# toonsegers/verifiable_mpc

Measured on AMD Instinct MI355X. Metric: Ed25519 MSM scalar-mults/sec, higher is better.
Workload: dtype u32 (255-bit modular integers as 10 limbs of 25.5 bits, 32x32->64 multiply-adds)

## Files before the change

verifiable_mpc_amd/csrc/msm.hip:

```cpp
#include <stdlib.h>

#include "common.h"
#include "fe25519.h"
#include "fr.h"
#include "ge25519.h"
#include "scan.h"
#include "quad.h"
#include "msm_sort.h"
#include "ptio.h"

#ifndef MSM_NIELS_STRIDE
#define MSM_NIELS_STRIDE 24
#endif
#ifndef MSM_REDUCE_WAVES
#define MSM_REDUCE_WAVES 2
#endif

__global__ void __launch_bounds__(MSM_BLOCK)
k_msm_prep(const uint32_t *__restrict__ aff, size_t n_main, const uint32_t *__restrict__ aff_extra,
           size_t n_total, uint32_t *__restrict__ niels) {
    size_t i = (size_t)blockIdx.x * blockDim.x + threadIdx.x;
    if (i >= n_total) return;
    const uint32_t *src = (i < n_main) ? aff + 16 * i : aff_extra + 16 * (i - n_main);
    ge_aff a;
// ... 364 lines not shown

extern "C" int vmpc_msm_dev(vmpc_ctx *ctx, const void *scalars, const void *affine_points, size_t n,
                            const void *extra_scalars, const void *extra_affine_points,
                            size_t n_extra, void *out_ext, void *out_affine) {
    if (!ctx || (n && (!scalars || !affine_points)) || (n_extra && (!extra_scalars || !extra_affine_points)))
        return VMPC_E_INVAL;
    if (!out_ext && !out_affine) return VMPC_E_INVAL;
    VMPC_HIP_CHECK(hipSetDevice(ctx->device));
    hipStream_t st = ctx->stream;
    size_t n_total = n + n_extra;
    if (n_total == 0) {
        uint32_t id_ext[32] = {0}, id_aff[16] = {0};
        id_ext[8] = 1; id_ext[16] = 1; id_aff[8] = 1;
        if (out_ext) VMPC_HIP_CHECK(hipMemcpyAsync(out_ext, id_ext, 128, hipMemcpyHostToDevice, st));
        if (out_affine) VMPC_HIP_CHECK(hipMemcpyAsync(out_affine, id_aff, 64, hipMemcpyHostToDevice, st));
        VMPC_HIP_CHECK(hipStreamSynchronize(st));
        return VMPC_OK;
    }
    if (n_total >= (1ull << 31) / 16) return VMPC_E_INVAL;
    msm_plan p;
    msm_make_plan(ctx, n, n_extra, 253, p, &ED25519_L);
    msm_ws w;
    msm_layout(p, w, nullptr, NIELS_WORDS * 4, EXT_WORDS * 4);
    VMPC_CHECK(vmpc_ws_reserve(ctx, w.total));
    msm_layout(p, w, (char *)ctx->ws, NIELS_WORDS * 4, EXT_WORDS * 4);

    {
        vmpc_stage_scope s(ctx, "msm_prep");
        k_msm_prep<<<(unsigned)((n_total + MSM_BLOCK - 1) / MSM_BLOCK), MSM_BLOCK, 0, st>>>(
            (const uint32_t *)affine_points, n, (const uint32_t *)extra_affine_points, n_total, w.entries);
        VMPC_KERNEL_CHECK();
    }
    VMPC_CHECK(msm_sort_stage(ctx, p, w, scalars, n, extra_scalars, ED25519_L));
    return msm_accumulate(ctx, p, w, w.entries, out_ext, out_affine);
}

bool msm_short_fits(const vmpc_ctx *ctx, size_t table_n, size_t table_extra, size_t m, int rows, int c, int K,
                    const void *out_ext, const void *out_affine);
int msm_short_batch(vmpc_ctx *ctx, const void *table, size_t table_n, size_t table_extra, const void *const *scalars,
                    size_t m, const void *const *extra_scalars, int K, void *out_ext, const msm_modulus &modulus);

static int msm_table_window(const vmpc_ctx *ctx) {
    const int o = ctx->window_override;
    return (o == 4 || o == 8 || o == 16) ? o : 16;
}
static size_t msm_table_stride(size_t n_points, int rows = 16) {
    return rows == MSM_WIDE_ROWS ? (n_points + 8191) & ~(size_t)8191 : (n_points + 7) & ~(size_t)7;
}
static bool msm_table_rows_ok(int rows) {
    return rows == 1 || rows == 2 || rows == 4 || rows == 8 || rows == 16 || rows == MSM_WIDE_ROWS;
}
static int msm_table_row_bits(int rows) { return rows == MSM_WIDE_ROWS ? MSM_WIDE_C : 256 / rows; }

__global__ void __launch_bounds__(MSM_BLOCK, 2)
k_msm_table_build(const uint32_t *__restrict__ aff, size_t n_main, const uint32_t *__restrict__ aff_extra,
                  size_t n_total, size_t stride, int rows, size_t col_begin, uint32_t *__restrict__ table) {
    size_t i = col_begin + (size_t)blockIdx.x * blockDim.x + threadIdx.x;
    if (i >= stride) return;
    if (i >= n_total) {
        ge_niels z;
        z.ymx = fe_one();
        z.ypx = fe_one();
        z.t2d = fe_zero();
        for (int r = 0; r < rows; r++) niels_st_line(table + NIELS_WORDS * ((size_t)r * stride + i), z);
        return;
    }
    const uint32_t *src = (i < n_main) ? aff + 16 * i : aff_extra + 16 * (i - n_main);
    ge_aff a;
    a.x = fe_ld8(src);
    a.y = fe_ld8(src + 8);
    niels_st_line(table + NIELS_WORDS * i, ge_niels_from_affine(a));
    ge_ext q = ge_ext_from_affine(a);
    const int dbl_per_row = rows == MSM_WIDE_ROWS ? MSM_WIDE_C : 256 / rows;
    fe run = fe_one();
    for (int r = 1; r < rows; r++) {
        for (int k = 0; k < dbl_per_row; k++) q = ge_dbl(q);
        run = fe_mul(run, q.Z);
        uint32_t *slot = table + NIELS_WORDS * ((size_t)r * stride + i);
        fe_st8(slot, q.X);
        fe_st8(slot + 8, q.Y);
        fe_st8(slot + 16, q.Z);
        fe_st8(slot + 24, run);
    }
    if (rows > 1) {
        fe inv = fe_inv(run);
        for (int r = rows - 1; r >= 1; r--) {
            uint32_t *slot = table + NIELS_WORDS * ((size_t)r * stride + i);
            const fe Z = fe_ld8(slot + 16);
            const fe prev = r > 1 ? fe_ld8(table + NIELS_WORDS * ((size_t)(r - 1) * stride + i) + 24) : fe_one();
            const fe zi = fe_mul(inv, prev);
            inv = fe_mul(inv, Z);
            ge_aff b;
            b.x = fe_canon(fe_mul(fe_ld8(slot), zi));
            b.y = fe_canon(fe_mul(fe_ld8(slot + 8), zi));
            niels_st_line(slot, ge_niels_from_affine(b));
        }
    }
}

extern "C" int vmpc_msm_table_bytes(size_t n, size_t n_extra, int rows, size_t *bytes) {
    if (!bytes || n + n_extra == 0 || n + n_extra > ((size_t)1 << 26) || !msm_table_rows_ok(rows)) return VMPC_E_INVAL;
    *bytes = (size_t)rows * msm_table_stride(n + n_extra, rows) * NIELS_WORDS * 4;
    return VMPC_OK;
}

extern "C" int vmpc_msm_table_build_dev(vmpc_ctx *ctx, const void *affine_points, size_t n,
                                        const void *extra_affine_points, size_t n_extra, int rows, void *table) {
    if (!ctx || !table || (n && !affine_points) || (n_extra && !extra_affine_points) || n + n_extra == 0 ||
        n + n_extra > ((size_t)1 << 26) || !msm_table_rows_ok(rows))
        return VMPC_E_INVAL;
    VMPC_HIP_CHECK(hipSetDevice(ctx->device));
    const size_t stride = msm_table_stride(n + n_extra, rows);
    vmpc_stage_scope s(ctx, "msm_table_build");
    k_msm_table_build<<<(unsigned)((stride + MSM_BLOCK - 1) / MSM_BLOCK), MSM_BLOCK, 0, ctx->stream>>>(
        (const uint32_t *)affine_points, n, (const uint32_t *)extra_affine_points, n + n_extra, stride, rows, 0,
        (uint32_t *)table);
    VMPC_KERNEL_CHECK();
    return VMPC_OK;
}

int vmpc_msm_table_build_extras(vmpc_ctx *ctx, size_t n, const void *extra_affine_points, size_t n_extra, int rows,
                                void *table) {
    const size_t stride = msm_table_stride(n + n_extra, rows);
    k_msm_table_build<<<(unsigned)((stride - n + MSM_BLOCK - 1) / MSM_BLOCK), MSM_BLOCK, 0, ctx->stream>>>(
        nullptr, n, (const uint32_t *)extra_affine_points, n + n_extra, stride, rows, n, (uint32_t *)table);
    VMPC_KERNEL_CHECK();
    return VMPC_OK;
}

static int msm_table_batch_wide(vmpc_ctx *ctx, const void *table, size_t table_n, size_t table_extra,
                                const void *const *scalars, size_t m, const void *const *extra_scalars, int K,
                                void *out_ext, void *out_affine) {
    const size_t stride = msm_table_stride(table_n + table_extra, MSM_WIDE_ROWS);
    if (stride > ((size_t)1 << 22)) return VMPC_E_INVAL;
    msm_plan p;
    p.n_main = p.n_total = (size_t)MSM_WIDE_ROWS * stride;
    p.n_extra = 0;
    p.scalar_bits = 253;
    p.c = MSM_WIDE_C;
    p.period = 1;
    p.W = K;
    p.top_row = -1;
    p.top_max_b = 0;
    p.wide = 1;
    p.row_stride = stride;
    p.chunks_per_row = (int)(stride / 8192);
    p.col_bits = 1;
    while (((size_t)1 << p.col_bits) < stride) p.col_bits++;
    msm_plan_geometry(ctx, p);
    msm_ws w;
    msm_layout(p, w, nullptr, 0, EXT_WORDS * 4);
    VMPC_CHECK(vmpc_ws_reserve(ctx, w.total));
    msm_layout(p, w, (char *)ctx->ws, 0, EXT_WORDS * 4);
    VMPC_CHECK(msm_recode_wide_batch(ctx, scalars, m, extra_scalars, K, table_n, table_extra, stride, (int32_t *)w.digits,
                                     p.n_pad, ED25519_L));
    VMPC_CHECK(msm_sort_digits(ctx, p, w));
    return msm_accumulate(ctx, p, w, (const uint32_t *)table, out_ext, out_affine);
}

static int msm_table_batch(vmpc_ctx *ctx, const void *table, size_t table_n, size_t table_extra, int rows,
                           const void *const *scalars, size_t m, const void *const *extra_scalars, int K,
                           void *out_ext, void *out_affine) {
    if (!ctx || !table || m > table_n || (m && !scalars) || table_n + table_extra == 0 || K < 1 || K > 16 ||
        table_n + table_extra > ((size_t)1 << 26) || !msm_table_rows_ok(rows) || (!out_ext && !out_affine))
        return VMPC_E_INVAL;
    VMPC_HIP_CHECK(hipSetDevice(ctx->device));
    for (int k = 0; k < K; k++)
        if (m && !scalars[k]) return VMPC_E_INVAL;
    if (msm_short_fits(ctx, table_n, table_extra, m, rows, msm_table_window(ctx), K, out_ext, out_affine)) {
        if (ctx->short_backoff > 0) ctx->short_backoff--;
        else return msm_short_batch(ctx, table, table_n, table_extra, scalars, m, extra_scalars, K, out_ext, ED25519_L);
    }
    if (rows == MSM_WIDE_ROWS)
        return msm_table_batch_wide(ctx, table, table_n, table_extra, scalars, m, extra_scalars, K, out_ext, out_affine);
    const size_t stride = msm_table_stride(table_n + table_extra);
    msm_plan p;
    p.n_main = p.n_total = (size_t)rows * stride;
    p.n_extra = 0;
    p.scalar_bits = 253;
    p.c = msm_table_window(ctx);
    const int windows = 256 / p.c;
    p.period = windows / rows;
    p.W = K * p.period;
    p.top_row = -1;
    p.top_max_b = 0;
    if (rows == 1) {
        msm_plan q;
        msm_make_plan(ctx, p.n_total, 0, 253, q, &ED25519_L);
        if (q.c == p.c && q.W == p.period) {
            p.top_row = q.top_row;
            p.top_max_b = q.top_max_b;
        }
    }
    msm_plan_geometry(ctx, p);
    msm_ws w;
    msm_layout(p, w, nullptr, 0, EXT_WORDS * 4);
    VMPC_CHECK(vmpc_ws_reserve(ctx, w.total));
    msm_layout(p, w, (char *)ctx->ws, 0, EXT_WORDS * 4);
    for (int k = 0; k < K; k++)
        if (m && !scalars[k]) return VMPC_E_INVAL;
    VMPC_CHECK(msm_recode_rows_batch(ctx, scalars, m, extra_scalars, K, table_n, table_extra, stride, w.digits,
                                     (size_t)p.period * p.n_pad, p.c, windows, rows, ED25519_L));
    VMPC_CHECK(msm_sort_digits(ctx, p, w));
    return msm_accumulate(ctx, p, w, (const uint32_t *)table, out_ext, out_affine);
}

extern "C" int vmpc_msm_table_dev(vmpc_ctx *ctx, const void *table, size_t table_n, size_t table_extra, int rows,
                                  const void *scalars, size_t m, const void *extra_scalars, void *out_ext,
                                  void *out_affine) {
    const void *sc[1] = {scalars}, *ex[1] = {extra_scalars};
    return msm_table_batch(ctx, table, table_n, table_extra, rows, sc, m, extra_scalars ? ex : nullptr, 1, out_ext,
                           out_affine);
}

extern "C" int vmpc_msm_table_batch_dev(vmpc_ctx *ctx, const void *table, size_t table_n, size_t table_extra, int rows,
                                        const void *const *scalars, size_t m, const void *const *extra_scalars,
                                        int batch, void *out_ext, void *out_affine) {
    return msm_table_batch(ctx, table, table_n, table_extra, rows, scalars, m, extra_scalars, batch, out_ext, out_affine);
}

int vmpc_normalize_launch(vmpc_ctx *ctx, const void *proj, size_t n, void *out_affine);

#define FB_C 8
#define FB_W 32
#define FB_D 128

__global__ void __launch_bounds__(64)
k_fb_bases(const uint32_t *__restrict__ base_aff, uint32_t *__restrict__ bases ) {
    if (threadIdx.x != 0 || blockIdx.x != 0) return;
    ge_aff a;
    a.x = fe_ld8(base_aff);
    a.y = fe_ld8(base_aff + 8);
    ge_ext q = ge_ext_from_affine(a);
    for (int w = 0; w < FB_W; w++) {
        ext_st(bases + EXT_WORDS * w, q);
        for (int k = 0; k < FB_C; k++) q = ge_dbl(q);
    }
}

__global__ void __launch_bounds__(MSM_BLOCK)
k_fb_table(const uint32_t *__restrict__ bases, uint32_t *__restrict__ table ) {
    const int t = blockIdx.x * blockDim.x + threadIdx.x;
    if (t >= FB_W * FB_D) return;
    const int w = t / FB_D, d = t % FB_D + 1;
    const ge_ext b = ext_ld(bases + EXT_WORDS * w);
    ge_ext r = ge_ext_identity();
    for (int k = 7; k >= 0; k--) {
        r = ge_dbl(r);
        if ((d >> k) & 1) r = ge_add(r, b);
    }
    niels_st_line(table + NIELS_WORDS * t, ge_niels_from_affine(ge_ext_to_affine(r)));
}

__global__ void __launch_bounds__(MSM_BLOCK)
k_fb_apply(const uint32_t *__restrict__ table, const uint32_t *__restrict__ sc, size_t n, msm_modulus mod,
           uint32_t *__restrict__ status, uint32_t *__restrict__ out_proj) {
    size_t i = (size_t)blockIdx.x * blockDim.x + threadIdx.x;
    if (i >= n) return;
    uint32_t s[8];
    load_u32x8(s, sc + 8 * i);
    {
        bool ge = true;
#pragma unroll
        for (int k = 7; k >= 0; k--) {
            if (s[k] != mod.v[k]) {
                ge = s[k] > mod.v[k];
                break;
            }
        }
        if (ge) atomicAdd(&status[VMPC_ST_NONCANON], 1u);
    }
    ge_ext acc = ge_ext_identity();
    uint32_t carry = 0;
#pragma unroll 1
    for (int w = 0; w < FB_W; w++) {
        uint32_t raw = ((s[w >> 2] >> (8 * (w & 3))) & 0xffu) + carry;
        int d;
        if (raw > FB_D) {
            d = (int)raw - 256;
            carry = 1;
        } else {
            d = (int)raw;
            carry = 0;
        }
        if (d != 0) {
            const uint32_t idx = (uint32_t)w * FB_D + (uint32_t)((d < 0 ? -d : d) - 1);
            acc = ge_madd(acc, ge_niels_select_neg(niels_ld_line(table + NIELS_WORDS * idx), d < 0));
        }
    }
    fe_st8(out_proj + 24 * i, acc.X);
    fe_st8(out_proj + 24 * i + 8, acc.Y);
    fe_st8(out_proj + 24 * i + 16, acc.Z);
}

extern "C" int vmpc_fixed_base_dev(vmpc_ctx *ctx, const void *base_affine, const void *scalars, size_t n,
                                   void *out_affine) {
    if (!ctx || !base_affine || (n && (!scalars || !out_affine))) return VMPC_E_INVAL;
    if (n == 0) return VMPC_OK;
    VMPC_HIP_CHECK(hipSetDevice(ctx->device));
    hipStream_t st = ctx->stream;
    const size_t bases_bytes = vmpc_align((size_t)FB_W * EXT_WORDS * 4);
    const size_t table_bytes = vmpc_align((size_t)FB_W * FB_D * NIELS_WORDS * 4);
    const size_t proj_bytes = vmpc_align(n * 96);
    VMPC_CHECK(vmpc_ws_reserve(ctx, bases_bytes + table_bytes + proj_bytes + 1024));
    uint32_t *bases = (uint32_t *)vmpc_ws_take(ctx, bases_bytes);
    uint32_t *table = (uint32_t *)vmpc_ws_take(ctx, table_bytes);
    uint32_t *proj = (uint32_t *)vmpc_ws_take(ctx, proj_bytes);
    vmpc_stage_scope s(ctx, "fixed_base");
    k_fb_bases<<<1, 64, 0, st>>>((const uint32_t *)base_affine, bases);
// ... 49 lines not shown
```

verifiable_mpc_amd/csrc/msm_sort.h:

```cpp
#pragma once
#include "common.h"

#define MSM_MAX_C 16
#define MSM_WIDE_C 20
#define MSM_WIDE_ROWS 13
#define MSM_BLOCK 256
#define MSM_SORT_BLOCK 1024
#define MSM_SEG 64
#define MSM_SEG_LOG2 6
#define MSM_FINISH_SERIAL 32
#ifndef MSM_REDUCE_CHUNKS
#define MSM_REDUCE_CHUNKS 4096
#endif

struct msm_plan {
    size_t n_main, n_extra, n_total;
    int scalar_bits;
    int c, W, nb, nb1;
    int seg_shift;
    int balanced;
    int LB;
    int NC;
    int J;
    int idx_bits;
    int fine_in_entry;
    int period;
    int top_row;
    uint32_t top_max_b;
    int LB_top;
    size_t n_pad;
    int chunks;
    int chunk_len;
    int red_blocks;
    int wide = 0;
    int chunks_per_row = 0;
    int col_bits = 0;
    size_t row_stride = 0;
    int fine_cap = 12288;
};
inline size_t msm_seg_len(const msm_plan &p) { return (size_t)1 << (MSM_SEG_LOG2 + p.seg_shift); }


struct msm_ws {
    uint32_t *entries;
    uint32_t *hist1;
    size_t hist1_n;
    uint32_t *stage1;
    uint32_t *counts, *starts, *sorted;
    uint32_t *buckets;
    uint32_t *partials;
    uint32_t *nseg, *seg_starts, *block_hist, *block_base, *heavy_list, *ctrl;
    uint32_t *seg_partial;
    uint2 *tasks;
    int16_t *digits;
    void *scan_ws;
    size_t total;
    uint32_t plan_blocks;
    size_t t_max;
};

struct msm_modulus {
    uint32_t v[8];
};

void msm_make_plan(vmpc_ctx *ctx, size_t n_main, size_t n_extra, int scalar_bits, msm_plan &p,
                   const msm_modulus *modulus = nullptr);
void msm_plan_geometry(vmpc_ctx *ctx, msm_plan &p);
void msm_layout(const msm_plan &p, msm_ws &w, char *base, size_t entry_bytes, size_t acc_bytes);
bool msm_reduce_tree_fits(const msm_plan &p);
int msm_reduce_tree_split(const msm_plan &p);
int msm_reduce_tree(vmpc_ctx *ctx, const msm_plan &p, msm_ws &w, hipStream_t st, void *out_packed);
int msm_sort_stage(vmpc_ctx *ctx, const msm_plan &p, msm_ws &w, const void *scalars, size_t n,
                   const void *extra_scalars, const msm_modulus &modulus);
int msm_sort_digits(vmpc_ctx *ctx, const msm_plan &p, msm_ws &w);
int msm_recode_wide_batch(vmpc_ctx *ctx, const void *const *scalars, size_t n_main, const void *const *extra_scalars,
                          int K, size_t extra_pos, size_t n_extra, size_t row_stride, int32_t *digits32,
                          size_t digits_per_commitment, const msm_modulus &modulus);
int msm_recode_rows(vmpc_ctx *ctx, const void *scalars, size_t n_main, const void *extra_scalars,
                    size_t extra_pos, size_t n_extra, size_t n_pad, int16_t *digits, int c, int W, int rows,
                    const msm_modulus &modulus);
int msm_recode_rows_batch(vmpc_ctx *ctx, const void *const *scalars, size_t n_main, const void *const *extra_scalars,
                          int K, size_t extra_pos, size_t n_extra, size_t n_pad, int16_t *digits,
                          size_t digits_per_commitment, int c, int W, int rows, const msm_modulus &modulus);

static inline int msm_ilog2(int v) {
    int r = 0;
    while ((1 << r) < v) r++;
    return r;
}

__host__ __device__ __forceinline__ uint32_t msm_seg_count(uint32_t cnt, uint32_t seg_log) {
    return (cnt + (1u << seg_log) - 1u) >> seg_log;
}
__device__ __forceinline__ void msm_seg_range(uint32_t cnt, uint32_t ns, uint32_t sidx, uint32_t seg, int balanced,
                                              uint32_t &off, uint32_t &len) {
    if (ns <= 1) {
        off = 0;
        len = cnt;
        return;
    }
    if (!balanced) {
        off = sidx * seg;
        len = cnt - off < seg ? cnt - off : seg;
        return;
    }
    const uint32_t q = cnt / ns, r = cnt - q * ns;
    off = sidx * q + (sidx < r ? sidx : r);
    len = q + (sidx < r ? 1u : 0u);
}

__device__ __forceinline__ size_t msm_bucket_slot(uint32_t ci, int nb1) {
    uint32_t w = ci / (uint32_t)nb1;
    return (size_t)ci - w - 1;
}
```

verifiable_mpc_amd/csrc/msm_sort.hip:

```cpp
#include "common.h"
#include "msm_sort.h"
#include "scan.h"

#define SORT_T 8192
#define SORT_BLOCK 1024
#define SORT_WAVES (SORT_BLOCK / 64)
#define SORT_FINE_CAP 12288

__device__ __forceinline__ uint32_t msm_seg_class(uint32_t rem, int seg_shift) {
    return seg_shift > 0 ? (rem + (1u << seg_shift) - 1u) >> seg_shift : rem;
}

__device__ __forceinline__ void load_u32x8(uint32_t dst[8], const uint32_t *src) {
    const uint4 *p = reinterpret_cast<const uint4 *>(src);
    uint4 a = p[0], b = p[1];
    dst[0] = a.x; dst[1] = a.y; dst[2] = a.z; dst[3] = a.w;
    dst[4] = b.x; dst[5] = b.y; dst[6] = b.z; dst[7] = b.w;
}

struct msm_recode_batch {
    const uint32_t *sc[16];
    const uint32_t *sc_extra[16];
};

__device__ __forceinline__ void
msm_recode_term(const uint32_t *__restrict__ sc, size_t n_main, const uint32_t *__restrict__ sc_extra,
                size_t extra_pos, size_t n_extra, size_t n_pad, int16_t *__restrict__ digits, int c, int W,
                int wpr, size_t set_stride, const msm_modulus &mod, uint32_t *__restrict__ status) {
    size_t i = (size_t)blockIdx.x * blockDim.x + threadIdx.x;
    if (i >= n_pad) return;
    const uint32_t *src = nullptr;
    if (i < n_main) src = sc + 8 * i;
    else if (sc_extra && i >= extra_pos && i < extra_pos + n_extra) src = sc_extra + 8 * (i - extra_pos);
    if (!src) {
        for (int w = 0; w < W; w++) digits[(size_t)(w % wpr) * set_stride + (size_t)(w / wpr) * n_pad + i] = 0;
        return;
    }
    uint32_t s[8];
    load_u32x8(s, src);
    {
        bool ge = true;
#pragma unroll
        for (int k = 7; k >= 0; k--) {
            if (s[k] != mod.v[k]) {
                ge = s[k] > mod.v[k];
                break;
            }
        }
        if (ge) {
            atomicAdd(&status[VMPC_ST_NONCANON], 1u);
#pragma unroll
            for (int k = 0; k < 8; k++) s[k] = 0;
        }
    }
    const uint32_t mask = (1u << c) - 1u;
    const uint32_t half = 1u << (c - 1);
    uint32_t carry = 0;
    for (int w = 0; w < W; w++) {
        uint32_t raw = (s[0] & mask) + carry;
        int32_t d;
        if (raw >= half) {
            d = (int32_t)raw - (int32_t)(1u << c);
            carry = 1;
        } else {
            d = (int32_t)raw;
            carry = 0;
        }
        digits[(size_t)(w % wpr) * set_stride + (size_t)(w / wpr) * n_pad + i] = (int16_t)d;
#pragma unroll
        for (int k = 0; k < 7; k++) s[k] = (s[k] >> c) | (s[k + 1] << (32 - c));
        s[7] >>= c;
    }
}

__global__ void __launch_bounds__(MSM_BLOCK)
k_msm_recode(const uint32_t *__restrict__ sc, size_t n_main, const uint32_t *__restrict__ sc_extra,
             size_t extra_pos, size_t n_extra, size_t n_pad, int16_t *__restrict__ digits, int c, int W,
             int wpr, size_t set_stride, msm_modulus mod, uint32_t *__restrict__ status) {
    msm_recode_term(sc, n_main, sc_extra, extra_pos, n_extra, n_pad, digits, c, W, wpr, set_stride, mod, status);
}

__global__ void __launch_bounds__(MSM_BLOCK)
k_msm_recode_batch(msm_recode_batch b, size_t n_main, size_t extra_pos, size_t n_extra, size_t n_pad,
                   int16_t *__restrict__ digits, size_t digits_per_commitment, int c, int W, int wpr,
                   size_t set_stride, msm_modulus mod, uint32_t *__restrict__ status) {
    msm_recode_term(b.sc[blockIdx.y], n_main, b.sc_extra[blockIdx.y], extra_pos, n_extra, n_pad,
                    digits + (size_t)blockIdx.y * digits_per_commitment, c, W, wpr, set_stride, mod, status);
}

__global__ void __launch_bounds__(MSM_BLOCK)
k_msm_recode_wide(msm_recode_batch b, size_t n_main, size_t extra_pos, size_t n_extra, size_t row_stride,
                  int32_t *__restrict__ digits, size_t digits_per_commitment, msm_modulus mod,
                  uint32_t *__restrict__ status) {
    const size_t i = (size_t)blockIdx.x * blockDim.x + threadIdx.x;
    if (i >= row_stride) return;
    const uint32_t *sc = b.sc[blockIdx.y], *sc_extra = b.sc_extra[blockIdx.y];
    int32_t *out = digits + (size_t)blockIdx.y * digits_per_commitment + i;
    const uint32_t *src = nullptr;
    if (i < n_main) src = sc + 8 * i;
    else if (sc_extra && i >= extra_pos && i < extra_pos + n_extra) src = sc_extra + 8 * (i - extra_pos);
    if (!src) {
#pragma unroll
        for (int r = 0; r < MSM_WIDE_ROWS; r++) out[(size_t)r * row_stride] = 0;
        return;
    }
    uint32_t s[9];
    load_u32x8(s, src);
    s[8] = 0;
    {
        bool ge = true;
#pragma unroll
        for (int k = 7; k >= 0; k--) {
            if (s[k] != mod.v[k]) {
                ge = s[k] > mod.v[k];
                break;
            }
        }
        if (ge) {
            atomicAdd(&status[VMPC_ST_NONCANON], 1u);
#pragma unroll
            for (int k = 0; k < 8; k++) s[k] = 0;
        }
    }
    if (mod.v[7] == 0x10000000u && (s[7] >> 16) != 0) {
        const uint32_t k = ((((uint32_t)i * 2654435761u) >> 16) * 121u) >> 16;
        uint64_t c2 = 0;
#pragma unroll
        for (int w = 0; w < 8; w++) {
            c2 += (uint64_t)s[w] + (uint64_t)k * mod.v[w];
            s[w] = (uint32_t)c2;
            c2 >>= 32;
        }
        s[8] = (uint32_t)c2;
    }
    uint64_t carry = 0;
#pragma unroll
    for (int k = 0; k < 9; k++) {
        uint32_t hk = 0;
#pragma unroll
        for (int r = 0; r < MSM_WIDE_ROWS; r++)
            if ((19 + 20 * r) / 32 == k) hk |= 1u << ((19 + 20 * r) % 32);
        const uint64_t v = (uint64_t)s[k] + hk + carry;
        s[k] = (uint32_t)v;
        carry = v >> 32;
    }
#pragma unroll
    for (int r = 0; r < MSM_WIDE_ROWS; r++) {
        const int bit = 20 * r, k = bit / 32, sh = bit % 32;
        uint32_t f = s[k] >> sh;
        if (sh > 12) f |= s[k + 1] << (32 - sh);
        out[(size_t)r * row_stride] = (int32_t)(f & 0xfffffu) - (int32_t)(1u << 19);
    }
}

template <bool WIDE>
__device__ __forceinline__ void sort_load8(const int16_t *__restrict__ digits, size_t at, int d[8]) {
    if (WIDE) {
        const uint4 *p = reinterpret_cast<const uint4 *>(reinterpret_cast<const int32_t *>(digits) + at);
        const uint4 a = p[0], b = p[1];
        d[0] = (int)a.x; d[1] = (int)a.y; d[2] = (int)a.z; d[3] = (int)a.w;
        d[4] = (int)b.x; d[5] = (int)b.y; d[6] = (int)b.z; d[7] = (int)b.w;
    } else {
        const uint4 v = *reinterpret_cast<const uint4 *>(digits + at);
        const uint32_t word[4] = {v.x, v.y, v.z, v.w};
#pragma unroll
        for (int k = 0; k < 8; k++) d[k] = (int)(int16_t)(word[k >> 1] >> (16 * (k & 1)));
    }
}

__device__ __forceinline__ int sort_xcd_chunk(int x, int J, int xcd) {
    if (!xcd) return x;
    const int per = (J + 7) / 8;
    return (x & 7) * per + (x >> 3);
}

template <bool WIDE>
__global__ void __launch_bounds__(SORT_BLOCK)
k_sort_hist1(const int16_t *__restrict__ digits, size_t n_pad, int NC, int LB, int top_row, int period, int LB_top,
             int J, int xcd, uint32_t *__restrict__ hist1, uint32_t *__restrict__ ctrl) {
    extern __shared__ uint32_t lds[];
    const int j = WIDE ? sort_xcd_chunk(blockIdx.x, J, xcd) : (int)blockIdx.x, w = blockIdx.y;
    if (w % period == top_row) LB = LB_top;
    if (blockIdx.x == 0 && w == 0)
        for (int i = threadIdx.x; i < 16 + MSM_SEG * (int)gridDim.y; i += SORT_BLOCK) ctrl[i] = 0;
    if (WIDE && j >= J) return;
    for (int b = threadIdx.x; b < NC; b += SORT_BLOCK) lds[b] = 0;
    __syncthreads();
    const size_t i0 = (size_t)j * SORT_T + 8 * (size_t)threadIdx.x;
    if (i0 < n_pad) {
        int d[8];
        sort_load8<WIDE>(digits, (size_t)w * n_pad + i0, d);
#pragma unroll
        for (int k = 0; k < 8; k++)
            if (d[k] != 0) atomicAdd(&lds[((uint32_t)(d[k] < 0 ? -d[k] : d[k]) - 1u) >> LB], 1u);
    }
    __syncthreads();
    for (int b = threadIdx.x; b < NC; b += SORT_BLOCK) hist1[((size_t)w * NC + b) * J + j] = lds[b];
}

template <bool WIDE>
__global__ void __launch_bounds__(SORT_BLOCK)
k_sort_part1(const int16_t *__restrict__ digits, size_t n_pad, int NC, int LB, int top_row, int period, int LB_top,
             int J, int idx_bits, int chunks_per_row, int xcd, const uint32_t *__restrict__ gbase,
             uint32_t *__restrict__ out) {
    extern __shared__ uint32_t lds[];
    uint32_t *cnt = lds;
    uint32_t *lbase = lds + NC;
    uint32_t *gb = lds + 2 * NC;
    uint32_t *scratch = lds + 3 * NC;
    uint32_t *stage = lds + 3 * NC + 16;
    const int j = WIDE ? sort_xcd_chunk(blockIdx.x, J, xcd) : (int)blockIdx.x, w = blockIdx.y;
    if (WIDE && j >= J) return;
    if (w % period == top_row) LB = LB_top;
    for (int b = threadIdx.x; b < NC; b += SORT_BLOCK) {
        cnt[b] = 0;
        gb[b] = gbase[((size_t)w * NC + b) * J + j];
    }
    __syncthreads();
    const size_t i0 = (size_t)j * SORT_T + 8 * (size_t)threadIdx.x;
    const size_t e0 = chunks_per_row ? i0 - (size_t)(j / chunks_per_row) * chunks_per_row * SORT_T : i0;
    uint32_t tag[8];
    int d[8] = {0, 0, 0, 0, 0, 0, 0, 0};
    if (i0 < n_pad) sort_load8<WIDE>(digits, (size_t)w * n_pad + i0, d);
#pragma unroll
    for (int k = 0; k < 8; k++) {
        tag[k] = 0xffffffffu;
        if (d[k] != 0) {
            const uint32_t cb = ((uint32_t)(d[k] < 0 ? -d[k] : d[k]) - 1u) >> LB;
            tag[k] = (cb << 16) | atomicAdd(&cnt[cb], 1u);
        }
    }
    __syncthreads();
    {
        uint32_t running = 0;
        for (int b0 = 0; b0 < NC; b0 += SORT_BLOCK) {
            const int b = b0 + (int)threadIdx.x;
            uint32_t v = b < NC ? cnt[b] : 0u, tot;
            uint32_t ex = vmpc_block_excl_scan<uint32_t>(v, &tot, scratch);
            if (b < NC) lbase[b] = running + ex;
            running += tot;
        }
    }
    __syncthreads();
    const uint32_t fmask = idx_bits < 31 ? (1u << LB) - 1u : 0u;
#pragma unroll
    for (int k = 0; k < 8; k++) {
        if (tag[k] != 0xffffffffu) {
            const uint32_t b = (uint32_t)(d[k] < 0 ? -d[k] : d[k]) - 1u;
            const uint32_t cb = tag[k] >> 16, pos = lbase[cb] + (tag[k] & 0xffffu);
            stage[pos] = (uint32_t)(e0 + k) | ((b & fmask) << (idx_bits & 31)) | (d[k] < 0 ? 0x80000000u : 0u);
            if (WIDE) stage[SORT_T + pos] = gb[cb] + (tag[k] & 0xffffu);
        }
    }
    __syncthreads();
    if (WIDE) {
        const uint32_t total = lbase[NC - 1] + cnt[NC - 1];
        for (uint32_t s = threadIdx.x; s < total; s += SORT_BLOCK) out[stage[SORT_T + s]] = stage[s];
        return;
    }
    const int wave = threadIdx.x >> 6, lane = threadIdx.x & 63;
    for (int b = wave; b < NC; b += SORT_WAVES) {
        const uint32_t len = cnt[b], lb = lbase[b], g = gb[b];
        for (uint32_t k = lane; k < len; k += 64) out[g + k] = stage[lb + k];
    }
}

template <bool FINE_IN_ENTRY>
__device__ __forceinline__ uint32_t sort_fine_of(uint32_t e, int idx_bits, uint32_t fmask,
                                                 const int16_t *__restrict__ drow) {
    if (FINE_IN_ENTRY) return (e >> idx_bits) & fmask;
    const int d = (int)drow[e & 0x7fffffffu];
    return ((uint32_t)(d < 0 ? -d : d) - 1u) & fmask;
}

__device__ __forceinline__ uint32_t sort_row_offset(const uint32_t *rb, int n_rows, uint32_t at, uint32_t row_stride) {
    uint32_t row = 0;
    for (int r = 1; r < n_rows; r++) row += rb[r] <= at ? 1u : 0u;
    return row * row_stride;
}

__device__ __forceinline__ int sort_row_lb(int w, int cb, int NC, int LB, int top_row, int period, int LB_top,
                                           int nb1, uint32_t *__restrict__ counts, uint32_t *__restrict__ nseg) {
    if (w % period != top_row) return LB;
    if (counts) {
        const uint32_t covered = (uint32_t)NC << LB_top, nb = (uint32_t)nb1 - 1u;
        for (uint32_t u = covered + cb * SORT_BLOCK + threadIdx.x; u < nb; u += NC * SORT_BLOCK) {
            counts[(size_t)w * nb1 + 1 + u] = 0;
            nseg[(size_t)w * nb1 + 1 + u] = 0;
        }
    }
    return LB_top;
}

template <bool FINE_IN_ENTRY, int CAP>
__global__ void __launch_bounds__(SORT_BLOCK, 8)
k_sort_fine(const uint32_t *__restrict__ in, const uint32_t *__restrict__ gbase, int NC, int W, int LB, int top_row,
            int period, int LB_top, int J, int idx_bits, int chunks_per_row, uint32_t row_stride, int nb1,
            const int16_t *__restrict__ digits, size_t n_pad,
            uint32_t *__restrict__ counts, uint32_t *__restrict__ starts, uint32_t *__restrict__ sorted,
            int seg_shift, int balanced, uint32_t *__restrict__ nseg, uint32_t *__restrict__ block_hist,
            uint32_t *__restrict__ heavy_list, uint32_t *__restrict__ seg_starts,
            uint32_t *__restrict__ ctrl ) {
    __shared__ uint32_t cnt[512], cur[512], scratch[16];
    __shared__ uint32_t lh[MSM_SEG + 1], heavy_n, heavy_segs, heavy_base, heavy_seg_base;
// ... 348 lines not shown
    p.n_main = n_main;
    p.n_extra = n_extra;
    p.n_total = n_main + n_extra;
    p.scalar_bits = scalar_bits;
    p.c = ctx->window_override ? ctx->window_override : msm_pick_window(p.n_total, scalar_bits);
    if (p.c < 4) p.c = 4;
    if (p.c > MSM_MAX_C) p.c = MSM_MAX_C;
    p.W = (scalar_bits + 2 + p.c - 1) / p.c;
    while (p.W > 64) {
        p.c++;
        p.W = (scalar_bits + 2 + p.c - 1) / p.c;
    }
    p.top_row = -1;
    p.top_max_b = 0;
    p.period = p.W;
    if (modulus) {
        p.top_row = p.W - 1;
        p.top_max_b = msm_top_max_bucket(*modulus, p.c, p.W);
    }
    msm_plan_geometry(ctx, p);
}

void msm_plan_geometry(vmpc_ctx *ctx, msm_plan &p) {
    if (p.period <= 0 || p.period > p.W) p.period = p.W;
    p.nb = 1 << (p.c - 1);
    p.nb1 = p.nb + 1;
    p.n_pad = (p.n_total + 7) & ~(size_t)7;
    p.idx_bits = 1;
    while (((size_t)1 << p.idx_bits) < p.n_pad) p.idx_bits++;
    const int nc_target = p.n_total >= ((size_t)1 << 22) ? 256 : 512;
    int lb = p.c - 1;
    if (lb > 9) lb = 9;
    while (lb > 0 && (p.nb >> lb) < nc_target && (p.n_total >> (p.c - 1 - lb)) > 8192) lb--;
    if (ctx->sort_fine_bits >= 0 && ctx->sort_fine_bits <= 9 && ctx->sort_fine_bits <= p.c - 1 &&
        (p.nb >> ctx->sort_fine_bits) <= 4096)
        lb = ctx->sort_fine_bits;
    p.fine_cap = SORT_FINE_CAP;
    if (p.wide) {
        lb = 9;
        while (lb > 6 && (p.n_total >> (p.c - 1 - lb)) > 14336) lb--;
        p.idx_bits = p.col_bits;
        p.fine_cap = 16384;
    }
    p.LB = lb;
    p.NC = p.nb >> lb;
    p.fine_in_entry = p.idx_bits + lb <= 31;
    p.LB_top = lb;
    if (p.top_row >= 0) {
        int lt = 0;
        while (lt < lb && (p.top_max_b >> lt) > (uint32_t)(p.NC - 1)) lt++;
        p.LB_top = lt;
    }
    p.J = (int)((p.n_pad + SORT_T - 1) / SORT_T);
    p.balanced = p.scalar_bits == 253 ? 1 : 0;
    const size_t work = ((size_t)p.W * p.n_total) >> ctx->plan_fill_shift;
    p.seg_shift = 0;
    while (p.seg_shift < 4 && (((size_t)MSM_SEG << p.seg_shift) << 18) < work) p.seg_shift++;
    while (p.seg_shift > ctx->seg_shift_min && (((size_t)MSM_SEG >> -(p.seg_shift - 1)) << 18) >= work)
        p.seg_shift--;
    int chunks = MSM_REDUCE_CHUNKS;
    while (chunks * 2 * p.W <= MSM_REDUCE_CHUNKS * 16 &&
           chunks * 2 <= (p.wide && ctx->reduce_max_chunks == 32768 ? 65536 : ctx->reduce_max_chunks))
        chunks *= 2;
    while (chunks * p.W > MSM_REDUCE_CHUNKS * 16 && chunks > 256) chunks /= 2;
    if (ctx->reduce_chunks_override >= 64) chunks = ctx->reduce_chunks_override;
    if (chunks > p.nb) chunks = p.nb;
    p.chunks = chunks;
    p.chunk_len = p.nb / chunks;
    p.red_blocks = (chunks + MSM_BLOCK - 1) / MSM_BLOCK;
}

void msm_layout(const msm_plan &p, msm_ws &w, char *base, size_t entry_bytes, size_t acc_bytes) {
    size_t off = 0;
    auto take = [&](size_t bytes) {
        size_t o = off;
        off += vmpc_align(bytes);
        return base ? (void *)(base + o) : (void *)nullptr;
    };
    size_t nbk = (size_t)p.W * p.nb1;
    w.entries = (uint32_t *)take(p.n_total * entry_bytes);
    w.digits = (int16_t *)take((size_t)p.W * p.n_pad * (p.wide ? 4 : 2));
    w.hist1_n = (size_t)p.W * p.NC * p.J;
    w.hist1 = (uint32_t *)take((w.hist1_n + 1) * 4);
    w.counts = (uint32_t *)take(nbk * 4);
    w.starts = (uint32_t *)take(nbk * 4);
    w.stage1 = (uint32_t *)take((size_t)p.W * p.n_total * 4);
    w.sorted = (uint32_t *)take((size_t)p.W * p.n_total * 4);
    w.buckets = (uint32_t *)take((size_t)p.W * p.nb * acc_bytes);
    w.partials = (uint32_t *)take((size_t)p.W * (3 * p.red_blocks + 4) * acc_bytes);
    size_t m_max = (size_t)p.W * p.n_total;
    size_t nonempty_max = m_max < (size_t)p.W * p.nb ? m_max : (size_t)p.W * p.nb;
    w.t_max = m_max / msm_seg_len(p) + nonempty_max;
    w.plan_blocks = (uint32_t)(p.W * p.NC);
    size_t hist_n = (size_t)MSM_SEG * w.plan_blocks;
    w.block_hist = (uint32_t *)take(hist_n * 4);
    w.block_base = (uint32_t *)take((size_t)MSM_SEG * p.W * 4);
    w.nseg = (uint32_t *)take(nbk * 4);
    w.seg_starts = (uint32_t *)take(nbk * 4);
    w.heavy_list = (uint32_t *)take(nbk * 4);
    w.ctrl = (uint32_t *)take((16 + (size_t)MSM_SEG * p.W) * 4);
    w.tasks = (uint2 *)take(w.t_max * 8);
    w.seg_partial = (uint32_t *)take(w.t_max * acc_bytes);
    size_t scan_n = hist_n;
    if (w.hist1_n > scan_n) scan_n = w.hist1_n;
    w.scan_ws = take(vmpc_scan_ws_bytes(scan_n, 4));
    w.total = off;
}

int msm_sort_stage(vmpc_ctx *ctx, const msm_plan &p, msm_ws &w, const void *scalars, size_t n,
                   const void *extra_scalars, const msm_modulus &modulus) {
    hipStream_t st = ctx->stream;
    const size_t n_total = p.n_total;
    const unsigned gb = (unsigned)((p.n_pad + MSM_BLOCK - 1) / MSM_BLOCK);
    {
        vmpc_stage_scope s(ctx, "msm_recode");
        k_msm_recode<<<gb, MSM_BLOCK, 0, st>>>((const uint32_t *)scalars, n,
                                              (const uint32_t *)extra_scalars, n, n_total - n, p.n_pad, w.digits, p.c,
                                              p.W, p.W, p.n_pad, modulus, ctx->d_status);
        VMPC_KERNEL_CHECK();
    }
    return msm_sort_digits(ctx, p, w);
}

int msm_recode_rows(vmpc_ctx *ctx, const void *scalars, size_t n_main, const void *extra_scalars,
                    size_t extra_pos, size_t n_extra, size_t n_pad, int16_t *digits, int c, int W, int rows,
                    const msm_modulus &modulus) {
    vmpc_stage_scope s(ctx, "msm_recode");
    const int wpr = W / rows;
    k_msm_recode<<<(unsigned)((n_pad + MSM_BLOCK - 1) / MSM_BLOCK), MSM_BLOCK, 0, ctx->stream>>>(
        (const uint32_t *)scalars, n_main, (const uint32_t *)extra_scalars, extra_pos, n_extra, n_pad, digits, c,
        W, wpr, (size_t)rows * n_pad, modulus, ctx->d_status);
    VMPC_KERNEL_CHECK();
    return VMPC_OK;
}

int msm_recode_rows_batch(vmpc_ctx *ctx, const void *const *scalars, size_t n_main, const void *const *extra_scalars,
                          int K, size_t extra_pos, size_t n_extra, size_t n_pad, int16_t *digits,
                          size_t digits_per_commitment, int c, int W, int rows, const msm_modulus &modulus) {
    vmpc_stage_scope s(ctx, "msm_recode");
    msm_recode_batch b;
    memset(&b, 0, sizeof b);
    for (int k = 0; k < K; k++) {
        b.sc[k] = (const uint32_t *)scalars[k];
        b.sc_extra[k] = extra_scalars ? (const uint32_t *)extra_scalars[k] : nullptr;
    }
    const int wpr = W / rows;
    k_msm_recode_batch<<<dim3((unsigned)((n_pad + MSM_BLOCK - 1) / MSM_BLOCK), K), MSM_BLOCK, 0, ctx->stream>>>(
        b, n_main, extra_pos, n_extra, n_pad, digits, digits_per_commitment, c, W, wpr, (size_t)rows * n_pad, modulus,
        ctx->d_status);
    VMPC_KERNEL_CHECK();
    return VMPC_OK;
}

int msm_recode_wide_batch(vmpc_ctx *ctx, const void *const *scalars, size_t n_main, const void *const *extra_scalars,
                          int K, size_t extra_pos, size_t n_extra, size_t row_stride, int32_t *digits32,
                          size_t digits_per_commitment, const msm_modulus &modulus) {
    vmpc_stage_scope s(ctx, "msm_recode");
    msm_recode_batch b;
    memset(&b, 0, sizeof b);
    for (int k = 0; k < K; k++) {
        b.sc[k] = (const uint32_t *)scalars[k];
        b.sc_extra[k] = extra_scalars ? (const uint32_t *)extra_scalars[k] : nullptr;
    }
    k_msm_recode_wide<<<dim3((unsigned)((row_stride + MSM_BLOCK - 1) / MSM_BLOCK), K), MSM_BLOCK, 0, ctx->stream>>>(
        b, n_main, extra_pos, n_extra, row_stride, digits32, digits_per_commitment, modulus, ctx->d_status);
    VMPC_KERNEL_CHECK();
    return VMPC_OK;
}

template <bool FINE_IN_ENTRY, int CAP>
static int msm_launch_fine(vmpc_ctx *ctx, const msm_plan &p, msm_ws &w) {
    hipStream_t st = ctx->stream;
    const unsigned grid = (unsigned)p.NC * (unsigned)p.W;
    const size_t dyn = CAP > SORT_FINE_CAP ? (size_t)CAP * 4 : 0;
    if (dyn && !ctx->sort_wide_ready) {
        VMPC_HIP_CHECK(hipFuncSetAttribute((const void *)k_sort_fine<FINE_IN_ENTRY, CAP>,
                                           hipFuncAttributeMaxDynamicSharedMemorySize, (int)dyn));
        VMPC_HIP_CHECK(hipFuncSetAttribute((const void *)k_sort_fine_big<FINE_IN_ENTRY, CAP>,
                                           hipFuncAttributeMaxDynamicSharedMemorySize, (int)dyn));
        ctx->sort_wide_ready = true;
    }
    k_sort_fine<FINE_IN_ENTRY, CAP><<<grid, SORT_BLOCK, dyn, st>>>(
        w.stage1, w.hist1, p.NC, p.W, p.LB, p.top_row, p.period, p.LB_top, p.J, p.idx_bits, p.chunks_per_row,
        (uint32_t)p.row_stride, p.nb1, w.digits, p.n_pad, w.counts, w.starts, w.sorted, p.seg_shift, p.balanced, w.nseg,
        w.block_hist, w.heavy_list, w.seg_starts, w.ctrl);
    k_sort_fine_big<FINE_IN_ENTRY, CAP><<<grid, SORT_BLOCK, dyn, st>>>(
        w.stage1, w.hist1, p.NC, p.W, p.LB, p.top_row, p.period, p.LB_top, p.J, p.idx_bits, p.chunks_per_row,
        (uint32_t)p.row_stride, p.nb1, w.digits, p.n_pad, w.starts, w.sorted, w.ctrl);
    VMPC_KERNEL_CHECK();
    return VMPC_OK;
}

int msm_sort_digits(vmpc_ctx *ctx, const msm_plan &p, msm_ws &w) {
    hipStream_t st = ctx->stream;
    if (p.wide && (!p.fine_in_entry || p.chunks_per_row <= 0 || p.J != p.chunks_per_row * MSM_WIDE_ROWS ||
                   p.n_pad != (size_t)p.J * SORT_T || p.row_stride != (size_t)p.chunks_per_row * SORT_T))
        return VMPC_E_INVAL;
    static const int xcd = getenv("VMPC_WIDE_XCD") ? atoi(getenv("VMPC_WIDE_XCD")) : 1;
    const dim3 chunk_grid(p.wide ? 8 * ((p.J + 7) / 8) : p.J, p.W);
    {
        vmpc_stage_scope s(ctx, "msm_hist");
        if (p.wide)
            k_sort_hist1<true><<<chunk_grid, SORT_BLOCK, (size_t)p.NC * 4, st>>>(w.digits, p.n_pad, p.NC, p.LB, p.top_row,
                                                                                p.period, p.LB_top, p.J, xcd, w.hist1, w.ctrl);
        else
            k_sort_hist1<false><<<chunk_grid, SORT_BLOCK, (size_t)p.NC * 4, st>>>(w.digits, p.n_pad, p.NC, p.LB, p.top_row,
                                                                                 p.period, p.LB_top, p.J, 0, w.hist1, w.ctrl);
        VMPC_KERNEL_CHECK();
        VMPC_CHECK((vmpc_exclusive_scan<uint32_t, uint32_t>(st, w.hist1, w.hist1, w.hist1_n, w.scan_ws,
                                                            w.hist1 + w.hist1_n)));
    }
    {
        vmpc_stage_scope s(ctx, "msm_part");
        const size_t lds_bytes = ((size_t)3 * p.NC + 16 + (p.wide ? 2 : 1) * SORT_T) * 4;
        if (p.wide) {
            if (lds_bytes > 48 * 1024)
                VMPC_HIP_CHECK(hipFuncSetAttribute((const void *)k_sort_part1<true>,
                                                   hipFuncAttributeMaxDynamicSharedMemorySize, (int)lds_bytes));
            k_sort_part1<true><<<chunk_grid, SORT_BLOCK, lds_bytes, st>>>(
                w.digits, p.n_pad, p.NC, p.LB, p.top_row, p.period, p.LB_top, p.J, p.idx_bits, p.chunks_per_row, xcd,
                w.hist1, w.stage1);
        } else {
            if (lds_bytes > 48 * 1024)
                VMPC_HIP_CHECK(hipFuncSetAttribute((const void *)k_sort_part1<false>,
                                                   hipFuncAttributeMaxDynamicSharedMemorySize, (int)lds_bytes));
            k_sort_part1<false><<<chunk_grid, SORT_BLOCK, lds_bytes, st>>>(
                w.digits, p.n_pad, p.NC, p.LB, p.top_row, p.period, p.LB_top, p.J, p.fine_in_entry ? p.idx_bits : 31, 0, 0,
                w.hist1, w.stage1);
        }
        VMPC_KERNEL_CHECK();
    }
    {
        vmpc_stage_scope s(ctx, "msm_sort");
        if (p.wide) VMPC_CHECK((msm_launch_fine<true, 16384>(ctx, p, w)));
        else if (p.fine_in_entry) VMPC_CHECK((msm_launch_fine<true, SORT_FINE_CAP>(ctx, p, w)));
        else VMPC_CHECK((msm_launch_fine<false, SORT_FINE_CAP>(ctx, p, w)));
    }
    {
        vmpc_stage_scope s(ctx, "msm_plan");
        if (p.W <= 8 && (size_t)p.W * p.NC <= 1024) {
            k_msm_ranks_classes<<<1, 1024, 0, st>>>(w.block_hist, p.NC, p.W, w.ctrl, w.block_base);
            VMPC_KERNEL_CHECK();
        } else {
            k_msm_ranks<<<p.W, 1024, 0, st>>>(w.block_hist, p.NC, p.W, w.ctrl);
            VMPC_KERNEL_CHECK();
            k_msm_classes<<<1, 1024, 0, st>>>(w.ctrl, p.W, w.block_base);
            VMPC_KERNEL_CHECK();
        }
        k_msm_plan2<<<w.plan_blocks, 512, 0, st>>>(w.counts, p.NC, p.W, 1 << p.LB, p.top_row, p.period, 1 << p.LB_top,
                                                  p.nb1, p.seg_shift, p.balanced, w.block_base, w.block_hist, w.tasks);
        VMPC_KERNEL_CHECK();
    }
    return VMPC_OK;
}
```

Baseline: 1.365 billion.

## Fuse wide scalar recoding with first-pass digit histogram

```diff
diff --git a/verifiable_mpc_amd/csrc/msm.hip b/verifiable_mpc_amd/csrc/msm.hip
--- a/verifiable_mpc_amd/csrc/msm.hip
+++ b/verifiable_mpc_amd/csrc/msm.hip
@@ -540,9 +540,7 @@
     msm_layout(p, w, nullptr, 0, EXT_WORDS * 4);
     VMPC_CHECK(vmpc_ws_reserve(ctx, w.total));
     msm_layout(p, w, (char *)ctx->ws, 0, EXT_WORDS * 4);
-    VMPC_CHECK(msm_recode_wide_batch(ctx, scalars, m, extra_scalars, K, table_n, table_extra, stride, (int32_t *)w.digits,
-                                     p.n_pad, ED25519_L));
-    VMPC_CHECK(msm_sort_digits(ctx, p, w));
+    VMPC_CHECK(msm_sort_wide_batch(ctx, p, w, scalars, m, extra_scalars, K, table_n, table_extra, ED25519_L));
     return msm_accumulate(ctx, p, w, (const uint32_t *)table, out_ext, out_affine);
 }
 
diff --git a/verifiable_mpc_amd/csrc/msm_sort.h b/verifiable_mpc_amd/csrc/msm_sort.h
--- a/verifiable_mpc_amd/csrc/msm_sort.h
+++ b/verifiable_mpc_amd/csrc/msm_sort.h
@@ -73,9 +73,9 @@
 int msm_sort_stage(vmpc_ctx *ctx, const msm_plan &p, msm_ws &w, const void *scalars, size_t n,
                    const void *extra_scalars, const msm_modulus &modulus);
 int msm_sort_digits(vmpc_ctx *ctx, const msm_plan &p, msm_ws &w);
-int msm_recode_wide_batch(vmpc_ctx *ctx, const void *const *scalars, size_t n_main, const void *const *extra_scalars,
-                          int K, size_t extra_pos, size_t n_extra, size_t row_stride, int32_t *digits32,
-                          size_t digits_per_commitment, const msm_modulus &modulus);
+int msm_sort_wide_batch(vmpc_ctx *ctx, const msm_plan &p, msm_ws &w, const void *const *scalars, size_t n_main,
+                        const void *const *extra_scalars, int K, size_t extra_pos, size_t n_extra,
+                        const msm_modulus &modulus);
 int msm_recode_rows(vmpc_ctx *ctx, const void *scalars, size_t n_main, const void *extra_scalars,
                     size_t extra_pos, size_t n_extra, size_t n_pad, int16_t *digits, int c, int W, int rows,
                     const msm_modulus &modulus);
diff --git a/verifiable_mpc_amd/csrc/msm_sort.hip b/verifiable_mpc_amd/csrc/msm_sort.hip
--- a/verifiable_mpc_amd/csrc/msm_sort.hip
+++ b/verifiable_mpc_amd/csrc/msm_sort.hip
@@ -88,68 +88,107 @@
                     digits + (size_t)blockIdx.y * digits_per_commitment, c, W, wpr, set_stride, mod, status);
 }
 
+__device__ __forceinline__ void
+msm_recode_wide_term(const uint32_t *__restrict__ sc, const uint32_t *__restrict__ sc_extra, size_t i, size_t n_main,
+                     size_t extra_pos, size_t n_extra, const msm_modulus &mod, uint32_t *__restrict__ status,
+                     int32_t d[MSM_WIDE_ROWS]) {
+    const uint32_t *src = nullptr;
+    if (i < n_main) src = sc + 8 * i;
+    else if (sc_extra && i >= extra_pos && i < extra_pos + n_extra) src = sc_extra + 8 * (i - extra_pos);
+    if (!src) {
+#pragma unroll
+        for (int r = 0; r < MSM_WIDE_ROWS; r++) d[r] = 0;
+        return;
+    }
+    uint32_t s[9];
+    load_u32x8(s, src);
+    s[8] = 0;
+    {
+        bool ge = true;
+#pragma unroll
+        for (int k = 7; k >= 0; k--) {
+            if (s[k] != mod.v[k]) {
+                ge = s[k] > mod.v[k];
+                break;
+            }
+        }
+        if (ge) {
+            atomicAdd(&status[VMPC_ST_NONCANON], 1u);
+#pragma unroll
+            for (int k = 0; k < 8; k++) s[k] = 0;
+        }
+    }
+    if (mod.v[7] == 0x10000000u && (s[7] >> 16) != 0) {
+        const uint32_t k = ((((uint32_t)i * 2654435761u) >> 16) * 121u) >> 16;
+        uint64_t c2 = 0;
+#pragma unroll
+        for (int w = 0; w < 8; w++) {
+            c2 += (uint64_t)s[w] + (uint64_t)k * mod.v[w];
+            s[w] = (uint32_t)c2;
+            c2 >>= 32;
+        }
+        s[8] = (uint32_t)c2;
+    }
+    uint64_t carry = 0;
+#pragma unroll
+    for (int k = 0; k < 9; k++) {
+        uint32_t hk = 0;
+#pragma unroll
+        for (int r = 0; r < MSM_WIDE_ROWS; r++)
+            if ((19 + 20 * r) / 32 == k) hk |= 1u << ((19 + 20 * r) % 32);
+        const uint64_t v = (uint64_t)s[k] + hk + carry;
+        s[k] = (uint32_t)v;
+        carry = v >> 32;
+    }
+#pragma unroll
+    for (int r = 0; r < MSM_WIDE_ROWS; r++) {
+        const int bit = 20 * r, k = bit / 32, sh = bit % 32;
+        uint32_t f = s[k] >> sh;
+        if (sh > 12) f |= s[k + 1] << (32 - sh);
+        d[r] = (int32_t)(f & 0xfffffu) - (int32_t)(1u << 19);
+    }
+}
+
 __global__ void __launch_bounds__(MSM_BLOCK)
 k_msm_recode_wide(msm_recode_batch b, size_t n_main, size_t extra_pos, size_t n_extra, size_t row_stride,
                   int32_t *__restrict__ digits, size_t digits_per_commitment, msm_modulus mod,
                   uint32_t *__restrict__ status) {
     const size_t i = (size_t)blockIdx.x * blockDim.x + threadIdx.x;
     if (i >= row_stride) return;
-    const uint32_t *sc = b.sc[blockIdx.y], *sc_extra = b.sc_extra[blockIdx.y];
     int32_t *out = digits + (size_t)blockIdx.y * digits_per_commitment + i;
-    const uint32_t *src = nullptr;
-    if (i < n_main) src = sc + 8 * i;
-    else if (sc_extra && i >= extra_pos && i < extra_pos + n_extra) src = sc_extra + 8 * (i - extra_pos);
-    if (!src) {
-#pragma unroll
-        for (int r = 0; r < MSM_WIDE_ROWS; r++) out[(size_t)r * row_stride] = 0;
-        return;
-    }
-    uint32_t s[9];
-    load_u32x8(s, src);
-    s[8] = 0;
-    {
-        bool ge = true;
-#pragma unroll
-        for (int k = 7; k >= 0; k--) {
-            if (s[k] != mod.v[k]) {
-                ge = s[k] > mod.v[k];
-                break;
-            }
-        }
-        if (ge) {
-            atomicAdd(&status[VMPC_ST_NONCANON], 1u);
-#pragma unroll
-            for (int k = 0; k < 8; k++) s[k] = 0;
-        }
-    }
-    if (mod.v[7] == 0x10000000u && (s[7] >> 16) != 0) {
-        const uint32_t k = ((((uint32_t)i * 2654435761u) >> 16) * 121u) >> 16;
-        uint64_t c2 = 0;
-#pragma unroll
-        for (int w = 0; w < 8; w++) {
-            c2 += (uint64_t)s[w] + (uint64_t)k * mod.v[w];
-            s[w] = (uint32_t)c2;
-            c2 >>= 32;
-        }
-        s[8] = (uint32_t)c2;
-    }
-    uint64_t carry = 0;
-#pragma unroll
-    for (int k = 0; k < 9; k++) {
-        uint32_t hk = 0;
-#pragma unroll
-        for (int r = 0; r < MSM_WIDE_ROWS; r++)
-            if ((19 + 20 * r) / 32 == k) hk |= 1u << ((19 + 20 * r) % 32);
-        const uint64_t v = (uint64_t)s[k] + hk + carry;
-        s[k] = (uint32_t)v;
-        carry = v >> 32;
-    }
-#pragma unroll
-    for (int r = 0; r < MSM_WIDE_ROWS; r++) {
-        const int bit = 20 * r, k = bit / 32, sh = bit % 32;
-        uint32_t f = s[k] >> sh;
-        if (sh > 12) f |= s[k + 1] << (32 - sh);
-        out[(size_t)r * row_stride] = (int32_t)(f & 0xfffffu) - (int32_t)(1u << 19);
+    int32_t d[MSM_WIDE_ROWS];
+    msm_recode_wide_term(b.sc[blockIdx.y], b.sc_extra[blockIdx.y], i, n_main, extra_pos, n_extra, mod, status, d);
+#pragma unroll
+    for (int r = 0; r < MSM_WIDE_ROWS; r++) out[(size_t)r * row_stride] = d[r];
+}
+
+__global__ void __launch_bounds__(SORT_BLOCK)
+k_msm_recode_hist_wide(msm_recode_batch b, size_t n_main, size_t extra_pos, size_t n_extra, size_t row_stride,
+                       int32_t *__restrict__ digits, size_t digits_per_commitment, msm_modulus mod,
+                       uint32_t *__restrict__ status, int NC, int LB, int J, int chunks_per_row,
+                       uint32_t *__restrict__ hist1, uint32_t *__restrict__ ctrl) {
+    extern __shared__ uint32_t lds[];
+    const int cc = blockIdx.x, w = blockIdx.y;
+    if (cc == 0 && w == 0)
+        for (int i = threadIdx.x; i < 16 + MSM_SEG * (int)gridDim.y; i += SORT_BLOCK) ctrl[i] = 0;
+    for (int k = threadIdx.x; k < MSM_WIDE_ROWS * NC; k += SORT_BLOCK) lds[k] = 0;
+    __syncthreads();
+    const uint32_t *sc = b.sc[w], *sc_extra = b.sc_extra[w];
+    for (int k = 0; k < SORT_T / SORT_BLOCK; k++) {
+        const size_t i = (size_t)cc * SORT_T + (size_t)k * SORT_BLOCK + threadIdx.x;
+        int32_t d[MSM_WIDE_ROWS];
+        msm_recode_wide_term(sc, sc_extra, i, n_main, extra_pos, n_extra, mod, status, d);
+        int32_t *out = digits + (size_t)w * digits_per_commitment + i;
+#pragma unroll
+        for (int r = 0; r < MSM_WIDE_ROWS; r++) {
+            out[(size_t)r * row_stride] = d[r];
+            if (d[r] != 0) atomicAdd(&lds[r * NC + (((uint32_t)(d[r] < 0 ? -d[r] : d[r]) - 1u) >> LB)], 1u);
+        }
+    }
+    __syncthreads();
+    for (int k = threadIdx.x; k < MSM_WIDE_ROWS * NC; k += SORT_BLOCK) {
+        const int r = k / NC, bin = k - r * NC;
+        hist1[((size_t)w * NC + bin) * J + (size_t)r * chunks_per_row + cc] = lds[k];
     }
 }
 
@@ -804,21 +843,6 @@
     return VMPC_OK;
 }
 
-int msm_recode_wide_batch(vmpc_ctx *ctx, const void *const *scalars, size_t n_main, const void *const *extra_scalars,
-                          int K, size_t extra_pos, size_t n_extra, size_t row_stride, int32_t *digits32,
-                          size_t digits_per_commitment, const msm_modulus &modulus) {
-    vmpc_stage_scope s(ctx, "msm_recode");
-    msm_recode_batch b;
-    memset(&b, 0, sizeof b);
-    for (int k = 0; k < K; k++) {
-        b.sc[k] = (const uint32_t *)scalars[k];
-        b.sc_extra[k] = extra_scalars ? (const uint32_t *)extra_scalars[k] : nullptr;
-    }
-    k_msm_recode_wide<<<dim3((unsigned)((row_stride + MSM_BLOCK - 1) / MSM_BLOCK), K), MSM_BLOCK, 0, ctx->stream>>>(
-        b, n_main, extra_pos, n_extra, row_stride, digits32, digits_per_commitment, modulus, ctx->d_status);
-    VMPC_KERNEL_CHECK();
-    return VMPC_OK;
-}
 
 template <bool FINE_IN_ENTRY, int CAP>
 static int msm_launch_fine(vmpc_ctx *ctx, const msm_plan &p, msm_ws &w) {
@@ -843,16 +867,34 @@
     return VMPC_OK;
 }
 
-int msm_sort_digits(vmpc_ctx *ctx, const msm_plan &p, msm_ws &w) {
+struct msm_wide_scalars {
+    msm_recode_batch b;
+    size_t n_main, extra_pos, n_extra;
+    const msm_modulus *modulus;
+};
+
+static int msm_sort_run(vmpc_ctx *ctx, const msm_plan &p, msm_ws &w, const msm_wide_scalars *fused) {
     hipStream_t st = ctx->stream;
     if (p.wide && (!p.fine_in_entry || p.chunks_per_row <= 0 || p.J != p.chunks_per_row * MSM_WIDE_ROWS ||
                    p.n_pad != (size_t)p.J * SORT_T || p.row_stride != (size_t)p.chunks_per_row * SORT_T))
         return VMPC_E_INVAL;
     static const int xcd = getenv("VMPC_WIDE_XCD") ? atoi(getenv("VMPC_WIDE_XCD")) : 1;
     const dim3 chunk_grid(p.wide ? 8 * ((p.J + 7) / 8) : p.J, p.W);
+    if (fused) {
+        vmpc_stage_scope s(ctx, "msm_recode");
+        const size_t lds_bytes = (size_t)MSM_WIDE_ROWS * p.NC * 4;
+        if (lds_bytes > 48 * 1024)
+            VMPC_HIP_CHECK(hipFuncSetAttribute((const void *)k_msm_recode_hist_wide,
+                                               hipFuncAttributeMaxDynamicSharedMemorySize, (int)lds_bytes));
+        k_msm_recode_hist_wide<<<dim3(p.chunks_per_row, p.W), SORT_BLOCK, lds_bytes, st>>>(
+            fused->b, fused->n_main, fused->extra_pos, fused->n_extra, p.row_stride, (int32_t *)w.digits, p.n_pad,
+            *fused->modulus, ctx->d_status, p.NC, p.LB, p.J, p.chunks_per_row, w.hist1, w.ctrl);
+        VMPC_KERNEL_CHECK();
+    }
     {
         vmpc_stage_scope s(ctx, "msm_hist");
-        if (p.wide)
+        if (fused) {
+        } else if (p.wide)
             k_sort_hist1<true><<<chunk_grid, SORT_BLOCK, (size_t)p.NC * 4, st>>>(w.digits, p.n_pad, p.NC, p.LB, p.top_row,
                                                                                 p.period, p.LB_top, p.J, xcd, w.hist1, w.ctrl);
         else
@@ -905,3 +947,29 @@
     }
     return VMPC_OK;
 }
+
+int msm_sort_digits(vmpc_ctx *ctx, const msm_plan &p, msm_ws &w) { return msm_sort_run(ctx, p, w, nullptr); }
+
+int msm_sort_wide_batch(vmpc_ctx *ctx, const msm_plan &p, msm_ws &w, const void *const *scalars, size_t n_main,
+                        const void *const *extra_scalars, int K, size_t extra_pos, size_t n_extra,
+                        const msm_modulus &modulus) {
+    if (!p.wide || K != p.W || K > 16) return VMPC_E_INVAL;
+    msm_wide_scalars f;
+    memset(&f.b, 0, sizeof f.b);
+    for (int k = 0; k < K; k++) {
+        f.b.sc[k] = (const uint32_t *)scalars[k];
+        f.b.sc_extra[k] = extra_scalars ? (const uint32_t *)extra_scalars[k] : nullptr;
+    }
+    f.n_main = n_main;
+    f.extra_pos = extra_pos;
+    f.n_extra = n_extra;
+    f.modulus = &modulus;
+    if ((size_t)MSM_WIDE_ROWS * p.NC * 4 <= 64 * 1024) return msm_sort_run(ctx, p, w, &f);
+    {
+        vmpc_stage_scope s(ctx, "msm_recode");
+        k_msm_recode_wide<<<dim3((unsigned)((p.row_stride + MSM_BLOCK - 1) / MSM_BLOCK), K), MSM_BLOCK, 0, ctx->stream>>>(
+            f.b, n_main, extra_pos, n_extra, p.row_stride, (int32_t *)w.digits, p.n_pad, modulus, ctx->d_status);
+        VMPC_KERNEL_CHECK();
+    }
+    return msm_sort_run(ctx, p, w, nullptr);
+}
```

New measurement: 1.350 billion. 1.1% lower.
